# Toptachamann/Linear_Programming_Solver

Measured on AMD Instinct MI355X. Metric: simplex_pivots_per_sec, higher is better.
Workload: dtype f64

## Files before the change

### include/lpx.h

```cpp
#ifndef LPX_H
#define LPX_H

#include <stddef.h>
#include <stdint.h>

#ifdef __cplusplus
extern "C" {
#endif

#define LPX_ABI_VERSION 5

typedef enum lpx_status {
  LPX_OPTIMAL = 0,
  LPX_UNBOUNDED = 1,
  LPX_INFEASIBLE = 2,
  LPX_AUX_UNBOUNDED = 3,
  LPX_NO_DEGENERATE_PIVOT = 4,
  LPX_BAD_ARGUMENT = 5,
  LPX_RESTORE_INDEX_FAULT = 6,
  LPX_DEVICE_ERROR = 7,
  LPX_DIVIDE_BY_ZERO = 8,
  LPX_PIVOT_LIMIT = 9
} lpx_status;

// ... 31 lines not shown
  LPX_OPT_CHAIN_FENCES = 6,
  LPX_OPT_SWEEP_ROWS = 7,
  LPX_OPT_NT = 8,
  LPX_OPT_BATCH = 9,
  LPX_OPT_CHAIN_TRACE = 10,
  LPX_OPT_UPDATE_U = 11,
  LPX_OPT_UPDATE_ROWS = 12,
  LPX_OPT_A2_OFFSET = 13,
  LPX_OPT_SWEEP_FORM = 14,
  LPX_OPT_MULTI_ONEHOP = 15,
  LPX_OPT_SWEEP_CUS = 16,
  LPX_OPT_CHAIN_CUS = 17,
  LPX_OPT_FUSED = 18,
  LPX_OPT_CHAIN_FORM = 19,
  LPX_OPT_FIXUP_SIDE = 20,
  LPX_OPT_COUNT = 21
} lpx_option;
int lpx_state_set_option(lpx_state* s, int32_t key, int64_t value);
int lpx_state_get_option(const lpx_state* s, int32_t key, int64_t* value);

typedef struct lpx_state_info {
  int32_t block;
  int32_t chain_wgs;
  int32_t chain_wgs_requested;
  int32_t chain_resident_max;
  int32_t chain_blocks_per_cu;
  int32_t chain_stream_masked;
  int32_t chain_xcd_mask;
  int32_t sweep_xcd_mask;
  int32_t overlapped;
  int32_t nontemporal;
  int32_t sweep_rows;
  int32_t sweep_kernel;
  int32_t multi_onehop;
  int32_t sweep_clock_mhz;
  int32_t sweep_cus;
  int32_t arith_fused;
} lpx_state_info;
int lpx_state_get_info(lpx_state* s, lpx_state_info* out);
const char* lpx_sweep_kernel_name(int32_t code);
int lpx_state_read_chain_trace(lpx_state* s, int64_t* ticks, int32_t cap, int32_t* ndecisions);
int lpx_state_read_chain_trace_fine(lpx_state* s, int64_t* ticks, int32_t cap, int32_t* ndecisions, int32_t* stamps);

int lpx_state_set_block(lpx_state* s, int32_t pivots_per_sweep);
int lpx_state_get_block(const lpx_state* s);

int lpx_simplex_loop(lpx_state* s, int64_t max_pivots, int64_t* pivots_done, int32_t* status,
                     int32_t* track_slot);

int lpx_state_read(lpx_state* s, double* A, int64_t lda, double* b, double* c, double* v,
                   int32_t* perm);
int lpx_state_dims(const lpx_state* s, int32_t* m_local, int32_t* n, int32_t* row0, int32_t* m_global);
// ... 137 lines not shown
```

### linear_programming_solver_amd/_lib.py

```python
import ctypes as C
import os

_HERE = os.path.dirname(os.path.abspath(__file__))
LIB_PATH = os.environ.get("LPX_LIB_PATH") or os.path.join(_HERE, "liblpx.so")

OPTIMAL, UNBOUNDED, INFEASIBLE, AUX_UNBOUNDED, NO_DEGENERATE_PIVOT, BAD_ARGUMENT, RESTORE_INDEX_FAULT, \
    DEVICE_ERROR, DIVIDE_BY_ZERO, PIVOT_LIMIT = range(10)
CAND_HEADER = 8
BATCH_LDS_BYTES = 163840
ROUTES = ("cold", "primal", "dual")
PRICING = {"reference": 0, "first-positive": 0, "dantzig": 1, 0: 0, 1: 1}

OPTIONS = {"block": 0, "chain": 1, "overlap": 2, "overlap_serial": 3, "overlap_mask": 4, "chain_wgs": 5,
           "chain_fences": 6, "sweep_rows": 7, "nt": 8, "batch": 9, "chain_trace": 10, "update_u": 11,
           "update_rows": 12, "a2_offset": 13, "sweep_form": 14, "multi_onehop": 15, "sweep_cus": 16, "chain_cus": 17,
           "fused": 18, "chain_form": 19, "fixup_side": 20}

DEFAULT_FUSED = None


def set_default_arithmetic(mode):
    global DEFAULT_FUSED
    if mode not in ("auto", "plain", "fused"):
        raise ValueError('arithmetic mode is "auto", "plain" or "fused"')
    prev = "auto" if DEFAULT_FUSED is None else "fused" if DEFAULT_FUSED else "plain"
    DEFAULT_FUSED = None if mode == "auto" else mode == "fused"
    return prev


dp = C.POINTER(C.c_double)
ip = C.POINTER(C.c_int32)
# ... 8 lines not shown
        ("objective_rounded", C.c_double),
        ("objective_text", C.c_char * 64),
        ("pivots_phase1", C.c_int64),
        ("pivots_phase2", C.c_int64),
        ("x0_slot", C.c_int32),
        ("reserved", C.c_int32),
        ("seconds_total", C.c_double),
        ("seconds_pivots", C.c_double),
    ]


class StateInfo(C.Structure):
    _fields_ = [(k, C.c_int32) for k in (
        "block", "chain_wgs", "chain_wgs_requested", "chain_resident_max", "chain_blocks_per_cu",
        "chain_stream_masked", "chain_xcd_mask", "sweep_xcd_mask", "overlapped", "nontemporal", "sweep_rows",
        "sweep_kernel", "multi_onehop", "sweep_clock_mhz", "sweep_cus", "arith_fused")]


class SolveOptions(C.Structure):
    _fields_ = [
        ("device", C.c_int32),
        ("has_variable_names", C.c_int32),
        ("max_pivots", C.c_int64),
        ("restore_order", ip),
        ("perm_out", ip),
        ("x_out", dp),
        ("keep_state", C.POINTER(C.c_void_p)),
        ("pricing", C.c_int32),
        ("restore_order_len", C.c_int32),
        ("fused", C.c_int32),
        ("reserved", C.c_int32),
# ... 129 lines not shown
```

### linear_programming_solver_amd/csrc/lpx_decisions.inc

```
constexpr int kMaxBlock = 32;

__global__ __launch_bounds__(256) void k_peek_multi(const double* __restrict__ A, int64_t ld,
                                                    const double* __restrict__ b, int m_local, int row0,
                                                    const double* __restrict__ prow_ring,
                                                    const double* __restrict__ col_ring, int64_t mp,
                                                    const LpxCtl* __restrict__ ring, int np,
                                                    double* __restrict__ col_out, double* __restrict__ col0_out,
                                                    RatioRow* __restrict__ partial,
                                                    const LpxCtl* __restrict__ ctl) {
  __shared__ RatioRow sh[4];
  __shared__ double sh_pe[kMaxBlock], sh_p[kMaxBlock], sh_bl[kMaxBlock];
  __shared__ int sh_e[kMaxBlock], sh_l[kMaxBlock];
  if (ctl->status != kRunning) return;
  const int en = ctl->e_next;
  if (en < 0) return;
  if ((int)threadIdx.x < np) {
    const LpxCtl& q = ring[threadIdx.x];
    sh_e[threadIdx.x] = q.e_cur;
    sh_l[threadIdx.x] = q.l - row0;
    sh_p[threadIdx.x] = q.p;
    sh_bl[threadIdx.x] = q.bl;
    sh_pe[threadIdx.x] = prow_ring[(int64_t)threadIdx.x * ld + en];
  }
  __syncthreads();
// ... 214 lines not shown
  int dantzig, fences;
  LpxCtl* host_snap;
  long long* dbg;
  unsigned* census;
  int shard_row0;
  int m_global;
  int n_dev, dev;
  int mail_slot0;
  MgMail* mail_peer[kMaxDevices];
  double* prow_peer[kMaxDevices];
  unsigned long long* arrive_peer[kMaxDevices];
  int onehop;
  double* candrow_peer[kMaxDevices];
  unsigned long long* arrive2_peer[kMaxDevices];
  unsigned spin_max;
  int diag;
};

template <int KB>
__device__ __forceinline__ int chain_restart(const unsigned long long* sh_mask) {
  if constexpr (KB > 32) {
    const unsigned long long hi = sh_mask[1], lo = sh_mask[0];
    return hi ? 127 - __clzll((long long)hi) : (lo ? 63 - __clzll((long long)lo) : -1);
  } else {
    const unsigned long long lo = sh_mask[0];
    return lo ? 63 - __clzll((long long)lo) : -1;
  }
}

template <bool MG, int KB>
// ... 606 lines not shown
  for (int k = 1; k < NW; ++k) {
    const MinRec o = sh[slot][k];
    if (o.ratio < r.ratio || (o.ratio == r.ratio && o.row < r.row)) r = o;
  }
  a = r.a;
  b = r.b;
  return RatioRow{r.ratio, r.row, 0};
}

constexpr int kChain2Threads = 256;
#ifdef LPX_CHAIN2_OWN_WT
#define LPX_OWN_STORE(p_, x_) st_agent((p_), (x_))
#else
#define LPX_OWN_STORE(p_, x_) (*(p_) = (x_))
#endif
template <int KB, int NT, bool MG>
__device__ __forceinline__ void block_chain2_body(const ChainArgs& P) {
  static_assert(KB == 32 || KB == 64 || KB == 128, "ring half of 32, 64 or 128 slots");
  static_assert(NT % 64 == 0 && NT >= 256 && NT >= 2 * KB + (KB == 128 ? 0 : 64), "lanes for the pending pivots and the loader lane");
  static_assert(KB <= 64 || !MG, "the shards decide at most kShardBlockMax pivots per block");
  constexpr int NC = 2 * KB / 8;
  constexpr int NH = (2 * KB + 63) / 64;
  constexpr int kWin = 8;
  __shared__ RatioRow sh_rr[NT / 64];
  __shared__ MinRec sh_rec[2][NT / 64];
  __shared__ unsigned sh_part[kChainMaxWgs * 8], sh_hand[8];
  __shared__ __attribute__((aligned(16))) double sh_pe[2 * KB], sh_cs[2 * KB], sh_dv[2 * KB], sh_p[2 * KB], sh_bl[2 * KB];
  __shared__ __attribute__((aligned(16))) int sh_e[2 * KB], sh_l[2 * KB];
  __shared__ int sh_fail;
#ifdef LPX_CHAIN2_FINE
#define LPX_C2_STAMP(k) if (P.dbg && lead) P.dbg[s * 16 + (k)] = wall_clock64();
#define LPX_C2_STRIDE 16
#else
#define LPX_C2_STAMP(k)
#define LPX_C2_STRIDE 8
#endif
  const int row0 = MG ? P.shard_row0 : 0;
  const double* __restrict__ A = P.A;
  const double* __restrict__ b = P.b;
  const int64_t ld = P.ld, mp = P.mp;
  const int n = P.n, m = P.m, nb = P.nb, n_old = P.n_old;
  LpxCtl* const ctl = P.ctl;
#ifdef LPX_CHAIN2_ONE_XCD
  if (blockIdx.x & 7u) return;
  const unsigned bid = blockIdx.x >> 3;
  const int G = gridDim.x >> 3;
#else
  const unsigned bid = blockIdx.x;
  const int G = gridDim.x;
#endif
  const int T = G * NT, tid = threadIdx.x, gid = bid * NT + tid;
  const bool lead = gid == 0;
  const bool book = bid == (unsigned)(G - 1) && tid == 0;
  if (tid == 0) {
    sh_fail = 0;
    if (P.census) P.census[bid] = xcc_id() + 1u;
  }
#ifdef LPX_CHAIN2_LAUNCH_STAMPS
  long long* const lst = P.dbg ? P.dbg + 8 * kBlockMax + 8 * ((P.hand_base / (unsigned)kBlockMax) & 1u) : nullptr;
  if (lst && lead) { lst[0] = wall_clock64(); lst[3] = P.hand_base / (unsigned)kBlockMax; }
#endif
  if (lead) st_agent(reinterpret_cast<int32_t*>(P.bar_next), 0);
  int e = ctl->e_next;
  if (ctl->status != kRunning || e < 0 || nb < 1) {
    if (book && nb >= 1) P.up[0].do_update = 0;
    if (book) chain_publish(ctl, P.host_snap);
    return;
  }
  if (tid < 2 * KB) {
    sh_pe[tid] = 0.0; sh_cs[tid] = 0.0; sh_dv[tid] = 0.0; sh_p[tid] = 1.0; sh_bl[tid] = 0.0;
    sh_e[tid] = -1; sh_l[tid] = -1;
  }
  lds_barrier();
  if (tid < n_old) {
    const LpxCtl& q = P.up_o[tid];
    sh_e[tid] = q.e_cur; sh_l[tid] = q.l; sh_p[tid] = q.p; sh_bl[tid] = q.bl;
  }
  int64_t pivots = ctl->pivots;
  const int64_t max_pivots = ctl->max_pivots;
  double v = ctl->v;
  int track = ctl->track, parity = ctl->parity;
  unsigned target = 0;
// ... 151 lines not shown
      if constexpr (NC > 2 * kWin) {
        if (L_a > 2 * kWin) {
          load_window_a(i, 2 * kWin);
          ladder_a(2 * kWin);
        }
        if (L_a > 3 * kWin) {
          load_window_a(i, 3 * kWin);
          ladder_a(3 * kWin);
        }
      }
      if (Lo_a >= L_a) a_mid = a;
      P.col0[(int64_t)s * mp + i] = a_mid;
      LPX_C2_STAMP(9)
      st_agent(&P.col[(int64_t)s * mp + i], a);
      LPX_OWN_STORE(&P.own_col[(int64_t)s * mp + i], a);
      if (i == gid) { a_first = a; b_first = bi; }
      const double rt = ratio_of(a, bi);
      if (rt < best.ratio) {
        best = RatioRow{rt, ig, 0};
        best_a = a;
        best_b = bi;
      }
      i += T;
      __builtin_amdgcn_sched_barrier(0);
      if (i < m) load_row(i);
    }
    LPX_C2_STAMP(10)
    const double pc = from32(sh_hand[1], sh_hand[2]);
    const unsigned xtag = P.hand_base + (unsigned)s;
    {
// ... 11 lines not shown
      }
      for (int idx = tid; idx < G * 8; idx += NT) {
        if ((idx & 7) == 7) continue;
        unsigned long long g;
        unsigned spins = 0;
        while ((unsigned)((g = __hip_atomic_load(&gran[idx], __ATOMIC_RELAXED, __HIP_MEMORY_SCOPE_AGENT)) >> 32) != xtag) {
          LPX_BARRIER_SLEEP;
          if (++spins > P.spin_max) { sh_fail = 1; break; }
        }
        sh_part[idx] = (unsigned)g;
      }
      if (P.fences & 2) __builtin_amdgcn_fence(__ATOMIC_ACQUIRE, "agent");
      lds_barrier();
      if (sh_fail) {
        if (book) { ctl->status = 7 ; ctl->reserved = sh_fail + 1000 * s; chain_publish(ctl, P.host_snap); }
        return;
      }
    }
    if (P.dbg && lead) P.dbg[s * LPX_C2_STRIDE + 3] = wall_clock64();

    RatioRow mine = rr_none();
    double mine_a = 0.0, mine_b = 0.0;
    for (int t = tid & 63; t < G; t += 64) {
      const unsigned* q = &sh_part[t * 8];
      const RatioRow o{from32(q[0], q[1]), (int)q[6], 0};
      if (o.ratio < mine.ratio || (o.ratio == mine.ratio && o.row < mine.row)) {
        mine = o;
        mine_a = from32(q[2], q[3]);
        mine_b = from32(q[4], q[5]);
      }
    }
// ... 40 lines not shown
      w = rr_wave_min_all(theirs);
      win_p = 0.0; win_b = 0.0;
      if (w.row != INT_MAX) {
        const int wl = __ffsll((long long)__ballot(theirs.row == w.row)) - 1;
        win_p = lane_f64(theirs_a, wl);
        win_b = lane_f64(theirs_b, wl);
      }
      lds_barrier();
      if (sh_fail) { if (book) { ctl->status = 7; ctl->reserved = sh_fail + 1000 * s; chain_publish(ctl, P.host_snap); } return; }
    }
    if (w.row == INT_MAX || !(w.ratio < kInf)) {
      if (book) {
        ctl->status = 1; ctl->do_update = 0; ctl->l = -1; ctl->ratio = w.ratio; P.up[s].do_update = 0;
        chain_publish(ctl, P.host_snap);
      }
      return;
    }
    if (max_pivots >= 0 && pivots >= max_pivots) {
      if (book) {
        ctl->status = 9 ; ctl->do_update = 0; P.up[s].do_update = 0;
        chain_publish(ctl, P.host_snap);
      }
      return;
    }
    LPX_C2_STAMP(12)
    const int l = w.row;
    const double p = win_p, raw_b = win_b;
    if (p == 0.0) {
      if (book) { ctl->status = 8; ctl->do_update = 0; P.up[s].do_update = 0; chain_publish(ctl, P.host_snap); }
      return;
    }
    int rb;
    {
      unsigned long long hit[NH];
#pragma unroll
      for (int h = 0; h < NH; ++h) hit[h] = __ballot(sh_l[h * 64 + (tid & 63)] == l);
      rb = top_bit_of(hit);
    }
    const bool owner = !MG || (l >= row0 && l < row0 + m);
    const int ll = l - row0;
    const int fo_b = rb < 0 ? 0 : (rb < KB ? rb + 1 : n_old);
    const int fn_b = rb >= KB ? rb - KB + 1 : 0;
    const int co0_b = fo_b >> 3, co1_b = fo_b < n_old ? (n_old + 7) >> 3 : co0_b;
    const int cn0_b = fn_b >> 3, cn1_b = fn_b < s ? (s + 7) >> 3 : cn0_b;
    const int Lo_b = owner ? co1_b - co0_b : 0, L_b = owner ? Lo_b + (cn1_b - cn0_b) : 0;
// ... 208 lines not shown
    int e_next = -2;
    have_rec = false;
    if (window) {
      if (tid < 5) {
        unsigned long long rec = 0;
        unsigned spins = 0;
        for (;;) {
          rec = __hip_atomic_load(&hand[tid], __ATOMIC_RELAXED, __HIP_MEMORY_SCOPE_AGENT);
          if ((unsigned)(rec >> 32) == xtag) break;
          LPX_BARRIER_SLEEP;
          if (++spins > P.spin_max) { sh_fail = 4; break; }
        }
        sh_hand[tid] = (unsigned)rec;
      }
      lds_barrier();
      if (sh_fail) { if (book) { ctl->status = 7; ctl->reserved = sh_fail + 1000 * s; chain_publish(ctl, P.host_snap); } return; }
      e_next = (int)sh_hand[0] - 2;
      have_rec = e_next >= 0;
    }
    if (e_next < 0) {
      const RatioRow w2 = rr_block_min2(cand, sh_rr);
      if (tid == 0) {
        st_agent(&P.partB[bid].ratio, w2.ratio);
        st_agent(&P.partB[bid].row, w2.row);
      }
      target += (unsigned)G;
      if (!grid_barrier(P.bar, target, &sh_fail, P.fences, P.spin_max)) {
        if (book) { ctl->status = 7; chain_publish(ctl, P.host_snap); }
        return;
      }
      RatioRow m2 = rr_none();
      if (tid < G) { m2.ratio = ld_agent(&P.partB[tid].ratio); m2.row = ld_agent(&P.partB[tid].row); }
      const RatioRow w3 = rr_block_min2(m2, sh_rr);
      e_next = (w3.row == INT_MAX) ? -1 : w3.row;
    }
    if (P.dbg && lead) P.dbg[s * LPX_C2_STRIDE + 7] = wall_clock64();
    pivots += 1;
    parity ^= 1;
    if (book) {
      ctl->v = v; ctl->p = p; ctl->bl = bl; ctl->pc = pc; ctl->ratio = w.ratio;
      ctl->e_cur = e; ctl->l = l; ctl->e_next = e_next; ctl->parity = parity; ctl->pivots = pivots;
      ctl->track = track; ctl->do_update = 1;
      if (e_next < 0) {
        ctl->status = 0 ;
        if (s + 1 < nb) P.up[s + 1].do_update = 0;
      }
    }
    if (e_next < 0 || s + 1 == nb) {
      if (book) chain_publish(ctl, P.host_snap);
      return;
    }
    e = e_next;
    lds_barrier();
  }
}
template <int KB, int NT, bool MG>
__global__ __launch_bounds__(NT) void k_block_chain2_t(const ChainArgs P) {
  static_assert(KB == 32 || KB == 64, "ring half of 32 or 64 slots");
  block_chain2_body<KB, NT, MG>(P);
}
template <int NT>
__global__ __launch_bounds__(NT) void k_block_decide128(const ChainArgs P) {
  block_chain2_body<128, NT, false>(P);
}
#undef LPX_C2_STAMP
#undef LPX_C2_STRIDE
#undef LPX_CHAIN_STEP_A
#undef LPX_CHAIN_STEP_B
#undef LPX_CHAIN_CHUNK_A
#undef LPX_CHAIN_CHUNK_B
#undef LPX_CHAIN_LIVE
```

### linear_programming_solver_amd/csrc/lpx_engine.cpp

```cpp
#include <hip/hip_runtime.h>

#include <algorithm>
#include <chrono>
#include <cmath>
#include <cstdio>
#include <cstdlib>
#include <cstring>
#include <string>
#include <vector>

#include "../../include/lpx.h"
#include "lpx_kernels.h"
#include "lpx_internal.h"

using lpxk::Buffers;
using lpxk::Geometry;
using lpxk::LpxCtl;
using lpxk::RatioRow;

thread_local std::string g_last_error;

int fail(int status, const std::string& msg) {
  g_last_error = msg;
  return status;
// ... 35 lines not shown
    {"LPX_CHAIN_FENCES", 2, 0, 3},
    {"LPX_SWEEP_ROWS", 0, 0, 8192},
    {"LPX_NT", -1, -1, 1},
    {"LPX_BATCH", 0, 0, 4096},
    {"LPX_CHAIN_TRACE", 0, 0, 1},
    {"LPX_U", 1, 1, 4},
    {"LPX_ROWS_PER_TILE", 2, 2, 256},
    {"LPX_A2_OFFSET", 512, 0, 1 << 20},
    {"LPX_SWEEP_FORM", 0, 0, 4},
    {"LPX_MULTI_ONEHOP", 0, 0, 1},
    {"LPX_SWEEP_CUS", 0, 0, 256},
    {"LPX_CHAIN_CUS", 0, 0, 16},
    {"LPX_FUSED", 2, 0, 2},
    {"LPX_CHAIN_FORM", 1, 0, 1},
    {"LPX_FIXUP_SIDE", 4, 0, 4},
};

static const int64_t* env_defaults() {
  static int64_t d[LPX_OPT_COUNT];
  static const bool once = [] {
    for (int k = 0; k < LPX_OPT_COUNT; k++) {
      const OptionSpec& sp = kOptionSpec[k];
      int64_t v = sp.dflt;
      const char* e = getenv(sp.env);
      if (e && *e) v = std::max(sp.lo, std::min(sp.hi, (int64_t)atoll(e)));
      d[k] = v;
    }
    return true;
  }();
  (void)once;
// ... 573 lines not shown
lpxk::BlockRing ring_half(const lpx_state* s, int h) {
  lpxk::BlockRing R = s->R;
  const int64_t o = (int64_t)h * lpxk::kBlockMax;
  R.prow += o * s->B.ld;
  R.row0 += o * s->B.ld;
  R.col += o * R.mp;
  R.col0 += o * R.mp;
  if (R.fix_col) R.fix_col += o * R.mp;
  if (R.fix_row) R.fix_row += o * s->B.ld;
  if (R.col_packed) R.col_packed += (int64_t)h * (R.mp / 4 + 1) * (4 * lpxk::kColPackedRowBytes / sizeof(double));
  if (R.tickets) R.tickets += (int64_t)h * lpxk::sweep_ticket_slots(s->B.ld) * 32;
  R.up += o;
  return R;
}

#ifndef LPX_CHAIN_CUS_PER_XCD
#define LPX_CHAIN_CUS_PER_XCD 4
#endif
static int chain_cus_per_xcd(const lpx_state* s, int per_xcd) {
  int k = LPX_CHAIN_CUS_PER_XCD;
  const int64_t work = std::max<int64_t>(s->m, s->B.ld);
  const double bytes = 8.0 * (double)s->m * (double)s->B.ld;
  if (!s->multi_shard && work > 8192 && bytes <= 1.5 * 1073741824.0) k = 8;
  if (!s->multi_shard && work > 8192 && s->B.fused) k = 8;
  if (s->opt[LPX_OPT_CHAIN_CUS] > 0) k = std::max(4, (int)s->opt[LPX_OPT_CHAIN_CUS] / 4 * 4);
  return std::max(1, std::min(k, (per_xcd - 1) / 4 * 4));
}
int ensure_overlap_streams(lpx_state* s) {
  if (s->ov_chain) return 0;
  hipDeviceProp_t prop;
// ... 93 lines not shown
  double* Abuf[2] = {s->B.A, s->A2};
  double* bbuf[2] = {s->B.b, s->b2};
  int64_t decided = 0;
  int nb_prev = 0, nblk = 0;
  const bool serial = s->opt[LPX_OPT_OVERLAP_SERIAL] != 0;
  int fix_mode = serial ? 0 : (int)s->opt[LPX_OPT_FIXUP_SIDE];
  if (fix_mode == 4) fix_mode = 8.0 * (double)s->m * (double)s->B.ld >= 2.0 * 1073741824.0 ? 2 : 0;
  if (fix_mode > 0 && ensure_fix_side(s, fix_mode) != 0) {
    (void)hipGetLastError();
    fix_mode = 0;
  }
  auto issue_block = [&](int k) -> int {
    const int nb = block_len(K, max_pivots, decided);
    if (nb <= 0) return 1;
    const int h = k & 1;
    Buffers Brd = s->B;
    if (serial) {
      if (k >= 1) HIP_TRY(hipStreamWaitEvent(s->ov_chain, s->ev_ov_sweep[h ^ 1], 0));
      Brd.A = Abuf[h];
      Brd.b = bbuf[h];
      s->info.chain_wgs = lpxk::launch_block_chain(Brd, s->R, s->n, s->m, nb, h, h ^ 1, 0, 1, s->chain_seq++, s->pricing == 1,
                                                   chain_wgs, fences, trace, d_snap + h, s->ov_chain, nullptr, s->ev_ov_chain[h]);
    } else {
      if (k >= 2) HIP_TRY(hipStreamWaitEvent(s->ov_chain, s->ev_ov_sweep[h], 0));
      Brd.A = Abuf[k == 0 ? 0 : (k - 1) & 1];
      Brd.b = bbuf[k == 0 ? 0 : (k - 1) & 1];
      s->info.chain_wgs = lpxk::launch_block_chain(Brd, s->R, s->n, s->m, nb, h, h ^ 1, k > 0 ? nb_prev : 0, k == 0,
                                                   s->chain_seq++, s->pricing == 1, chain_wgs, fences, trace, d_snap + h,
                                                   s->ov_chain, nullptr, s->ev_ov_chain[h]);
    }
    s->chain_nb_last = nb;
    if (max_pivots >= 0 && decided == max_pivots) {
      decided += nb;
      return 0;
    }
    HIP_TRY(hipStreamWaitEvent(s->ov_sweep, s->ev_ov_chain[h], 0));
    Buffers Bdst = s->B;
    Bdst.A = Abuf[h ^ 1];
    Bdst.b = bbuf[h ^ 1];
    const lpxk::FixSide side{fix_mode > 0 ? s->ov_fix[fix_mode] : nullptr, s->ev_ov_chain[h], s->ev_ov_fix[h], s->ev_ov_pack[h]};
    if (int rc = launch_sweep_profiled(s, nb, s->ov_sweep, Bdst, ring_half(s, h), Abuf[h], bbuf[h], fix_mode > 0 ? &side : nullptr,
                                       s->ev_ov_sweep[h])) return rc;
    decided += nb;
    nb_prev = nb;
    nblk = k + 1;
    return 0;
  };
  int rc = issue_block(0);
  if (rc == 1) rc = 0;
  for (int k = 1; rc == 0; k++) {
    const int r = issue_block(k);
    if (r != 0 && r != 1) { rc = r; break; }
    hipError_t e = hipEventSynchronize(s->ev_ov_chain[(k - 1) & 1]);
    if (e != hipSuccess) { rc = fail(LPX_DEVICE_ERROR, hipGetErrorString(e)); break; }
    if (h2[(k - 1) & 1].status != lpxk::kRunning || r == 1) break;
  }
  (void)hipEventRecord(s->ev_ov_join[1], s->ov_chain);
// ... 27 lines not shown
  int64_t decided = 0;
  const bool fused = s->opt[LPX_OPT_CHAIN] != 0 && s->row0 == 0 && s->m == s->m_global;
  const int64_t work = std::max<int64_t>(s->m, s->B.ld);
  const int auto_wgs = (int)std::min<int64_t>(64, std::max<int64_t>(1, (work + 255) / 256));
  const int chain_wgs = fused ? clamp_chain_wgs(s, s->opt[LPX_OPT_CHAIN_WGS] > 0 ? (int)s->opt[LPX_OPT_CHAIN_WGS] : auto_wgs,
                                                device_cus(s))
                              : 0;
  const int fences = (int)s->opt[LPX_OPT_CHAIN_FENCES];
  const bool trace = s->opt[LPX_OPT_CHAIN_TRACE] != 0;
  s->info.chain_stream_masked = 0;
  s->info.overlapped = 0;
  LpxCtl* d_snap = nullptr;
  if (fused) HIP_TRY(hipHostGetDevicePointer((void**)&d_snap, s->h_snap, 0));
  auto issue_block = [&](int slot) -> int {
    const int nb = block_len(K, max_pivots, decided);
    if (fused && nb > 0) {
      s->info.chain_wgs = lpxk::launch_block_chain(s->B, s->R, s->n, s->m, nb, 0, 0, 0, 1, s->chain_seq++, s->pricing == 1,
                                                   chain_wgs, fences, trace, d_snap + slot, s->stream);
      s->chain_nb_last = nb;
    } else {
      for (int k = 0; k < nb; k++) {
        lpxk::launch_block_peek(s->B, s->R, s->n, s->m, s->row0, k, s->d_cand, s->stream);
        lpxk::launch_block_decide(s->B, s->R, s->n, s->m_global, s->d_cand, 1, k, s->stream);
        if (s->pricing == 1) lpxk::launch_entering_dantzig(s->B, s->n, false, s->stream);
      }
    }
    const bool probe_only = max_pivots >= 0 && decided == max_pivots;
    decided += nb;
    if (nb > 0 && !probe_only) {
      if (int rc = launch_sweep_profiled(s, nb)) return rc;
    }
    if (!fused)
      HIP_TRY(hipMemcpyAsync(&h2[slot], s->B.ctl, sizeof(LpxCtl), hipMemcpyDeviceToHost, s->stream));
    HIP_TRY(hipEventRecord(evs[slot], s->stream));
    return 0;
  };
  int rc = issue_block(0);
  int cur = 0;
  while (rc == 0) {
    rc = issue_block(cur ^ 1);
    if (rc) break;
    hipError_t e = hipEventSynchronize(evs[cur]);
    if (e != hipSuccess) { rc = fail(LPX_DEVICE_ERROR, hipGetErrorString(e)); break; }
    if (h2[cur].status != lpxk::kRunning) break;
    cur ^= 1;
// ... 76 lines not shown
    HIP_TRY(hipStreamSynchronize(s->stream));
    std::vector<unsigned> h(lpxk::kChainMaxWgs + 2);
    HIP_TRY(hipMemcpy(h.data(), s->R.census, h.size() * sizeof(unsigned), hipMemcpyDeviceToHost));
    for (int w = 0; w < s->info.chain_wgs && w < (int)lpxk::kChainMaxWgs; w++)
      if (h[w]) s->info.chain_xcd_mask |= 1 << ((h[w] - 1) & 15);
    s->info.sweep_xcd_mask = (int32_t)h[lpxk::kChainMaxWgs];
  }
  s->info.sweep_clock_mhz = 0;
  if (s->R.clk) {
    long long c32[32] = {};
    HIP_TRY(hipStreamSynchronize(s->stream));
    HIP_TRY(hipMemcpy(c32, s->R.clk, sizeof c32, hipMemcpyDeviceToHost));
    std::vector<double> mhz;
    for (int x = 0; x < 8; x++) {
      const long long* c4 = c32 + 4 * x;
      if (c4[3] > c4[1] && c4[2] > c4[0] && c4[3] - c4[1] > 1000) {
        const double f = 100.0 * (double)(c4[2] - c4[0]) / (double)(c4[3] - c4[1]);
        if (f > 300.0 && f < 3500.0) mhz.push_back(f);
      }
    }
    if (!mhz.empty()) {
      std::sort(mhz.begin(), mhz.end());
      s->info.sweep_clock_mhz = (int32_t)(mhz[mhz.size() / 2] + 0.5);
    }
  }
  *out = s->info;
  return 0;
}

extern "C" const char* lpx_sweep_kernel_name(int32_t code) { return lpxk::sweep_kernel_name(code); }

// ... 358 lines not shown
```

### linear_programming_solver_amd/csrc/lpx_kernels.h

```cpp
#pragma once
#include <hip/hip_runtime.h>
#include <stdint.h>

namespace lpxk {

constexpr int kRunning = -1;
constexpr double kEps = 1e-9;
constexpr double kInf = 1e50;

struct RatioRow {
  double ratio;
  int32_t row;
  int32_t pad;
};

struct LpxCtl {
  double v;
  double p;
  double bl;
  double pc;
  double ratio;
  int32_t e_next;
  int32_t e_cur;
  int32_t l;
// ... 46 lines not shown
  unsigned* chain_bar;
  double* chain_own_col;
  double* chain_own_prow;
  double* chain_own_dvc;
  double* chain_own_b;
  int32_t* chain_own_rs;
  long long* chain_dbg;
  unsigned* census;
  double* fix_col;
  double* fix_row;
  double* col_packed;
  unsigned* tickets;
  unsigned* sweep_fail;
  long long* clk;
  const double* zeros;
  void* mg_mail;
  unsigned long long* mg_arrive;
  double* mg_candrow;
  unsigned long long* mg_arrive2;
};
struct MgPeers {
  int n_dev, dev;
  int row0, m_global;
  int mail_slot0;
  void* mail[kMaxDevices];
  double* prow[kMaxDevices];
  unsigned long long* arrive[kMaxDevices];
  int onehop;
  double* candrow[kMaxDevices];
  unsigned long long* arrive2[kMaxDevices];
  unsigned spin_max;
};
enum SweepKernel { kSweepNone = 0, kSweepTiles = 1, kSweepMulti = 2, kSweepSteady = 3, kSweepPipe64 = 4, kSweepDma = 5, kSweepPull = 6, kSweepPull64 = 7, kSweepOne64 = 8, kSweepMfma64 = 9, kSweepMfma642 = 10, kSweepMfma128 = 11 };
struct FixSide { hipStream_t stream; hipEvent_t ready, done, packed; };
constexpr int kColPackedRowBytes = 1024;
constexpr int kSweep128Ranges = 3;
struct RestoreEntry { int32_t is_basic; int32_t index; double k; };

constexpr int kBatchLdsMax = 163840;
constexpr int kBatchScratchBytes = 512;
struct BatchLayout {
  int64_t ld, b, c, v, perm, image, col;
  int64_t lds_bytes;
};
__host__ __device__ inline BatchLayout batch_layout(int64_t m, int64_t n) {
  BatchLayout L;
  L.ld = n | 1;
  L.b = m * L.ld;
  L.c = L.b + m;
  L.v = L.c + n;
  L.perm = (L.v + 2) & ~(int64_t)1;
// ... 114 lines not shown
```

### linear_programming_solver_amd/csrc/lpx_kernels.hip

```cpp
#include "lpx_kernels.h"

#include <hip/hip_ext.h>

#include <atomic>

#include <limits.h>
#include <stdint.h>
#include <stdlib.h>

#include <algorithm>
#include <type_traits>

#ifndef LPX_FUSED
#define LPX_FUSED 0
#endif

namespace lpxk {
#if LPX_FUSED
namespace fused {
#else
namespace plain {
#endif

typedef double d2 __attribute__((ext_vector_type(2)));
// ... 812 lines not shown
  const int64_t ho = half * K, oo = old_half * K;
  P.prow = R.prow + ho * B.ld; P.col = R.col + ho * R.mp; P.col0 = R.col0 + ho * R.mp; P.row0 = R.row0 + ho * B.ld;
  P.own_col = R.chain_own_col + ho * R.mp; P.own_prow = R.chain_own_prow + ho * B.ld;
  P.own_dvc = R.chain_own_dvc + ho * R.mp; P.up = R.up + ho;
  P.prow_o = R.prow + oo * B.ld; P.col_o = R.col + oo * R.mp;
  P.own_col_o = R.chain_own_col + oo * R.mp; P.own_prow_o = R.chain_own_prow + oo * B.ld;
  P.own_dvc_o = R.chain_own_dvc + oo * R.mp; P.up_o = R.up + oo;
  P.n_old = n_old; P.own_b = R.chain_own_b; P.b_from_tableau = b_from_tableau; P.nb = nb;
  P.own_rs_a = R.chain_own_rs; P.own_rs_b = R.chain_own_rs + R.mp;
  P.partA = reinterpret_cast<ChainPart*>(R.chain_part_a); P.partB = reinterpret_cast<RatioRow*>(R.chain_part_b);
  P.bar = R.chain_bar + 32 * (seq & 1); P.bar_next = R.chain_bar + 32 * ((seq + 1) & 1);
  P.hand = reinterpret_cast<unsigned long long*>(R.chain_bar + 64);
  P.hand_base = (unsigned)(seq + 1) * (unsigned)kBlockMax;
  P.dantzig = dantzig; P.fences = fences; P.host_snap = host_snap; P.dbg = trace ? R.chain_dbg : nullptr;
  P.spin_max = (mg && mg->spin_max) ? mg->spin_max : (1u << 22);
#ifdef LPX_DIAG_BUILD
  static const int chain_diag = getenv("LPX_CHAIN_DIAG") ? atoi(getenv("LPX_CHAIN_DIAG")) : 0;
  P.diag = chain_diag;
#endif
  P.census = R.census;
  if (mg) {
    P.shard_row0 = mg->row0; P.m_global = mg->m_global; P.n_dev = mg->n_dev; P.dev = mg->dev;
    P.mail_slot0 = mg->mail_slot0;
    P.onehop = mg->onehop;
    for (int d = 0; d < mg->n_dev && d < kMaxDevices; ++d) {
      P.mail_peer[d] = reinterpret_cast<MgMail*>(mg->mail[d]);
      P.prow_peer[d] = mg->prow[d] + ho * B.ld;
      P.arrive_peer[d] = mg->arrive[d];
      P.candrow_peer[d] = mg->candrow[d];
      P.arrive2_peer[d] = mg->arrive2[d];
// ... 85 lines not shown
#undef LPX_PRE_ONE64
#if LPX_FUSED
    hipLaunchKernelGGL(k_pack_multipliers_mfma, dim3(1), dim3(256), 0, s, R.col, R.mp, R.up, 0, 0, R.col_packed, R.tickets, 0, (long long*)nullptr, 0);
#ifdef LPX_WITH_VARIANTS
#define LPX_PRE_MFMA64(NT_, OOP_) \
    hipLaunchKernelGGL((k_sweep64_mfma<NT_, OOP_>), dim3(1), dim3(256), 0, s, A, A, ld, 0, R.prow, R.up, 0, 1, R.col_packed, R.tickets);
    LPX_EACH_NT_OOP(LPX_PRE_MFMA64)
#undef LPX_PRE_MFMA64
#endif
#define LPX_PRE_MFMA642(NT_, OOP_) \
    hipLaunchKernelGGL((k_sweep64_mfma2<NT_, OOP_>), dim3(1), dim3(256), 0, s, A, A, ld, 0, R.prow, R.up, 0, 1, R.col_packed, R.tickets, 33, (long long*)nullptr);
    LPX_EACH_NT_OOP(LPX_PRE_MFMA642)
#undef LPX_PRE_MFMA642
    hipLaunchKernelGGL(k_pack_multipliers_mfma128, dim3(1), dim3(256), 0, s, R.col, R.mp, R.up, 0, 0, R.col_packed, R.tickets, 0, (long long*)nullptr);
#define LPX_PRE_MFMA128(NT_, OOP_) \
    hipLaunchKernelGGL((k_sweep128_mfma<NT_, OOP_>), dim3(1), dim3(256), 0, s, A, A, ld, 0, R.prow, R.up, 0, 0, R.col_packed, R.tickets, 1);
    LPX_EACH_NT_OOP(LPX_PRE_MFMA128)
#undef LPX_PRE_MFMA128
#endif
  }
#undef LPX_PRE_PULL
#undef LPX_PRE_DMA
#undef LPX_PRE_PIPE
#undef LPX_PRE_STEADY
#undef LPX_PRE_MULTI
#undef LPX_PRE_T32
#undef LPX_PRE_T16
#undef LPX_PRE_T8
#undef LPX_PRE_T4
#undef LPX_PRE_T2
#undef LPX_PRE_TILES
// ... 135 lines not shown
  if (A_src) { if (nt) LPX_LAUNCH_MFMA64(true, true); else LPX_LAUNCH_MFMA64(false, true); }
  else { if (nt) LPX_LAUNCH_MFMA64(true, false); else LPX_LAUNCH_MFMA64(false, false); }
#undef LPX_LAUNCH_MFMA64
#else
  (void)G;
#endif
}
#endif

#if LPX_FUSED
static void launch_sweep128_mfma(const Buffers& B, const BlockRing& R, int m_local, int kmax, bool nt, const double* A_src,
                                 hipStream_t s, int cus, const FixSide* side, hipEvent_t t0, hipEvent_t t1) {
  const int nsub = (int)(B.ld / 64);
  const int ntiles = m_local / 16;
  const int nranges = std::max(1, std::min(kSweep128Ranges, ntiles));
  LPX_LAUNCH_STOP(k_pack_multipliers_mfma128, dim3(ntiles), dim3(256), pack_stream(side, s), pack_stop(side), R.col, R.mp, R.up, kmax,
                  ntiles, R.col_packed, R.tickets, 1 + nsub * nranges, R.clk);
  pack_done(side, s);
  const dim3 grid(std::max(1, std::min(2 * cus, nsub * nranges))), block(256);
#define LPX_LAUNCH_MFMA128(NT_, OOP_)                                                                                    \
  LPX_LAUNCH_TIMED((k_sweep128_mfma<NT_, OOP_>), grid, block, s, t0, t1, B.A, A_src, B.ld, m_local, R.prow, R.up, kmax, nsub, \
                   R.col_packed, R.tickets, nranges)
  if (A_src) { if (nt) LPX_LAUNCH_MFMA128(true, true); else LPX_LAUNCH_MFMA128(false, true); }
  else { if (nt) LPX_LAUNCH_MFMA128(true, false); else LPX_LAUNCH_MFMA128(false, false); }
#undef LPX_LAUNCH_MFMA128
}
#endif

static int choose_sweep_rows(int m_local, int64_t ld, int K, int cus) {
  const int64_t nstrips = (ld + 511) / 512;
  const int64_t slots = std::max(1, 2 * cus);
  const int prologue_rows = std::max(8, (K * 3) / 2);
  int best_rows = kSweepChunk;
  int64_t best_cost = INT64_MAX;
  const int max_rows = (int)std::min<int64_t>(4096, (((int64_t)1 << 32) - 1) / (ld * 8) / kSweepChunk * kSweepChunk);
  for (int rows = kSweepChunk; rows <= std::max(kSweepChunk, max_rows); rows += kSweepChunk) {
    const int64_t groups = (m_local + rows - 1) / rows;
// ... 52 lines not shown
  else side = nullptr;
  if (K <= 16) {
    bracket();
    int rows_per_tile = rows_per_wg <= 0 ? 16 : rows_per_wg;
    rows_per_tile = std::max(8, std::min(rows_per_tile, kSweepMaxRows)) & ~7;
    while (rows_per_tile > 8 && (int64_t)rows_per_tile * B.ld * 8 >= (int64_t)1 << 32) rows_per_tile -= 8;
    if (K <= 2) launch_sweep_tiles<2>(B, R, m_local, K, rows_per_tile, nt, A_src, s);
    else if (K <= 4) launch_sweep_tiles<4>(B, R, m_local, K, rows_per_tile, nt, A_src, s);
    else if (K <= 8) launch_sweep_tiles<8>(B, R, m_local, K, rows_per_tile, nt, A_src, s);
    else launch_sweep_tiles<16>(B, R, m_local, K, rows_per_tile, nt, A_src, s);
    rows_per_wg = rows_per_tile;
    used = kSweepTiles;
  } else if (K > 64) {
    bool mfma128 = false;
#if LPX_FUSED
    mfma128 = form != 3 && m_local % 16 == 0 && m_local >= 16 && B.ld % 512 == 0 && 16 * B.ld * 8 + 1024 < ((int64_t)1 << 32) &&
              R.tickets && R.col_packed;
#endif
    if (mfma128) {
#if LPX_FUSED
      timed_own = before_sweep && after_sweep;
      if (!timed_own) bracket();
      launch_sweep128_mfma(B, R, m_local, K, nt, A_src, s, cus, side, timed_own ? before_sweep : nullptr, timed_own ? after_sweep : nullptr);
#endif
      rows_per_wg = 16;
      used = kSweepMfma128;
    } else {
      bracket();
      int rows = choose_sweep_rows(m_local, B.ld, 32, cus);
      while (rows > kSweepChunk && (int64_t)rows * B.ld * 8 >= (int64_t)1 << 32) rows -= kSweepChunk;
      for (int slot0 = 0; slot0 < K; slot0 += 32) launch_sweep_k<32>(B, R, m_local, K, rows, nt, slot0 == 0 ? A_src : nullptr, s, 0, slot0);
      rows_per_wg = rows;
// ... 160 lines not shown
```

### linear_programming_solver_amd/csrc/lpx_sweeps.inc

```
constexpr int kSweepMaxRows = 128;
#ifndef LPX_SWEEP_NBUF
#define LPX_SWEEP_NBUF 2
#endif

__device__ __forceinline__ int ring_count(const LpxCtl* __restrict__ ring, int kcap, int kmax, int* sh_np) {
  if (threadIdx.x < 64) {
    const int lane = threadIdx.x;
    const bool ok = lane < kcap && lane < kmax && ring[lane].do_update != 0;
    const unsigned long long mask = __ballot(ok);
    if (lane == 0) *sh_np = (~mask == 0ull) ? 64 : (__ffsll((long long)~mask) - 1);
  }
  __syncthreads();
  return *sh_np;
}
__device__ __forceinline__ int ring_count128(const LpxCtl* __restrict__ ring, int kmax, int* sh_np) {
  if (threadIdx.x < 64) {
    const int lane = threadIdx.x;
    const unsigned long long m0 = __ballot(lane < kmax && ring[lane].do_update != 0);
    const unsigned long long m1 = __ballot(lane + 64 < kmax && ring[lane + 64].do_update != 0);
    const int n0 = (~m0 == 0ull) ? 64 : (__ffsll((long long)~m0) - 1);
    const int n1 = (~m1 == 0ull) ? 64 : (__ffsll((long long)~m1) - 1);
    if (lane == 0) *sh_np = n0 < 64 ? n0 : 64 + n1;
  }
  __syncthreads();
// ... 912 lines not shown
  for (int q = 0; q < 8; ++q) {
    const int idx = q * 256 + threadIdx.x;
    const int g = idx >> 6, l = idx & 63, k = l >> 4, i = l & 15;
    const int s = 4 * g + k;
    const double c = s < np ? col_ring[(int64_t)s * mp + (int64_t)tile * 16 + i] : 0.0;
    colM[(int64_t)tile * 2048 + (g >> 1) * 128 + 2 * l + (g & 1)] = -c;
  }
}
#define LPX_MFMA_FENCE __builtin_amdgcn_sched_barrier(0)
template <bool NT, bool OOP>
__global__ __launch_bounds__(256, 2) void k_sweep128_mfma(double* A, const double* Asrc,
                                                          int64_t ld, int m_local,
                                                          const double* __restrict__ prow_ring,
                                                          const LpxCtl* __restrict__ ring, int kmax, int nsub,
                                                          const double* colM,
                                                          unsigned* tickets, int nranges) {
  constexpr int NG = 32, CT = 4;
  constexpr int kRsrcWord3 = 0x00020000;
  constexpr int kAuxNt = NT ? 2 : 0;
  __shared__ __attribute__((aligned(16))) double sh_b[NG * CT * 64];
  __shared__ int sh_np, sh_chunk;
  const int np = ring_count128(ring, kmax, &sh_np);
  if (np < 1 && !OOP) return;
  const int lane = threadIdx.x & 63;
  const int wave = __builtin_amdgcn_readfirstlane((int)(threadIdx.x >> 6));
  const int rowblocks = m_local / 16;
  const int per_range = (rowblocks + nranges - 1) / nranges;
  const int nchunks = nsub * nranges;
  const int64_t row_bytes = ld * 8;
  const uint32_t rb32 = (uint32_t)row_bytes;
  const uint32_t off_c = (uint32_t)(lane >> 4) * rb32 + (uint32_t)(lane & 15) * 8u;
  const uint32_t off_a = (uint32_t)lane * 8u;
  int sub_loaded = -1;
  for (;;) {
    if (threadIdx.x == 0) sh_chunk = (int)atomicAdd(tickets, 1u);
    __syncthreads();
    const int chunk = __builtin_amdgcn_readfirstlane(sh_chunk);
    if (chunk >= nchunks) return;
    const int sub = chunk % nsub, range = chunk / nsub;
    const int rb0 = range * per_range;
    const int ntiles = min(rowblocks, rb0 + per_range) - rb0;
    if (sub != sub_loaded) {
      for (int q = wave; q < NG * CT; q += 4) {
        const int g = q / CT, ct = q % CT;
        const int s = 4 * g + (lane >> 4);
        sh_b[q * 64 + lane] = s < np ? prow_ring[(int64_t)s * ld + sub * 64 + ct * 16 + (lane & 15)] : 0.0;
      }
      sub_loaded = sub;
    }
    __syncthreads();
    if (ntiles > 0) {
      unsigned* const ctr = tickets + 32 * (1 + chunk);
      char* const dst_base = reinterpret_cast<char*>(A + sub * 64) + (int64_t)rb0 * 16 * row_bytes;
// ... 351 lines not shown
```

Baseline: 24470.

## Pack MFMA multipliers inside the decide chain kernel instead of a separate pack launch

When the fused chain form runs a 128-slot block on a single shard, the decide kernel now writes each negated pivot column directly into the packed MFMA column layout and resets the sweep tickets. On early exit it pads the unused slots with zeros. This lets the sweep skip the separate k_pack_multipliers_mfma128 launch and its stream/event handoff. In exchange, every column element costs an extra scattered store inside the latency-critical chain kernel. The change also moves clock sampling from the pack kernel into the sweep kernel and tightens a filter in the clock-rate estimate.

Result: no change. 24280 (-0.8%).

```diff
diff --git a/include/lpx.h b/include/lpx.h
--- a/include/lpx.h
+++ b/include/lpx.h
@@ -69,7 +69,8 @@
   LPX_OPT_FUSED = 18,
   LPX_OPT_CHAIN_FORM = 19,
   LPX_OPT_FIXUP_SIDE = 20,
-  LPX_OPT_COUNT = 21
+  LPX_OPT_PACK_IN_DECIDE = 21,
+  LPX_OPT_COUNT = 22
 } lpx_option;
 int lpx_state_set_option(lpx_state* s, int32_t key, int64_t value);
 int lpx_state_get_option(const lpx_state* s, int32_t key, int64_t* value);
@@ -91,6 +92,8 @@
   int32_t sweep_clock_mhz;
   int32_t sweep_cus;
   int32_t arith_fused;
+  int32_t pack_in_decide;
+  int32_t reserved;
 } lpx_state_info;
 int lpx_state_get_info(lpx_state* s, lpx_state_info* out);
 const char* lpx_sweep_kernel_name(int32_t code);
diff --git a/linear_programming_solver_amd/_lib.py b/linear_programming_solver_amd/_lib.py
--- a/linear_programming_solver_amd/_lib.py
+++ b/linear_programming_solver_amd/_lib.py
@@ -14,7 +14,7 @@
 OPTIONS = {"block": 0, "chain": 1, "overlap": 2, "overlap_serial": 3, "overlap_mask": 4, "chain_wgs": 5,
            "chain_fences": 6, "sweep_rows": 7, "nt": 8, "batch": 9, "chain_trace": 10, "update_u": 11,
            "update_rows": 12, "a2_offset": 13, "sweep_form": 14, "multi_onehop": 15, "sweep_cus": 16, "chain_cus": 17,
-           "fused": 18, "chain_form": 19, "fixup_side": 20}
+           "fused": 18, "chain_form": 19, "fixup_side": 20, "pack_in_decide": 21}
 
 DEFAULT_FUSED = None
 
@@ -53,7 +53,7 @@
     _fields_ = [(k, C.c_int32) for k in (
         "block", "chain_wgs", "chain_wgs_requested", "chain_resident_max", "chain_blocks_per_cu",
         "chain_stream_masked", "chain_xcd_mask", "sweep_xcd_mask", "overlapped", "nontemporal", "sweep_rows",
-        "sweep_kernel", "multi_onehop", "sweep_clock_mhz", "sweep_cus", "arith_fused")]
+        "sweep_kernel", "multi_onehop", "sweep_clock_mhz", "sweep_cus", "arith_fused", "pack_in_decide", "reserved")]
 
 
 class SolveOptions(C.Structure):
diff --git a/linear_programming_solver_amd/csrc/lpx_decisions.inc b/linear_programming_solver_amd/csrc/lpx_decisions.inc
--- a/linear_programming_solver_amd/csrc/lpx_decisions.inc
+++ b/linear_programming_solver_amd/csrc/lpx_decisions.inc
@@ -252,6 +252,9 @@
   double* candrow_peer[kMaxDevices];
   unsigned long long* arrive2_peer[kMaxDevices];
   unsigned spin_max;
+  double* colM;
+  unsigned* tickets;
+  int nctr;
   int diag;
 };
 
@@ -888,6 +891,14 @@
 #else
 #define LPX_OWN_STORE(p_, x_) (*(p_) = (x_))
 #endif
+__device__ __forceinline__ int64_t colm_index(int s, int i) {
+  return (int64_t)(i >> 4) * 2048 + (s >> 3) * 128 + 2 * ((s & 3) * 16 + (i & 15)) + ((s >> 2) & 1);
+}
+__device__ __forceinline__ void colm_pad(double* colM, int done, int gid, int T, int m) {
+  if (!colM || done >= 128) return;
+  for (int i = gid; i < m; i += T)
+    for (int u = done; u < 128; ++u) colM[colm_index(u, i)] = -0.0;
+}
 template <int KB, int NT, bool MG>
 __device__ __forceinline__ void block_chain2_body(const ChainArgs& P) {
   static_assert(KB == 32 || KB == 64 || KB == 128, "ring half of 32, 64 or 128 slots");
@@ -909,6 +920,7 @@
 #define LPX_C2_STAMP(k)
 #define LPX_C2_STRIDE 8
 #endif
+#define LPX_C2_LEAVE(done_) do { if constexpr (KB == 128) colm_pad(P.colM, (done_), gid, T, m); return; } while (0)
   const int row0 = MG ? P.shard_row0 : 0;
   const double* __restrict__ A = P.A;
   const double* __restrict__ b = P.b;
@@ -935,11 +947,15 @@
   if (lst && lead) { lst[0] = wall_clock64(); lst[3] = P.hand_base / (unsigned)kBlockMax; }
 #endif
   if (lead) st_agent(reinterpret_cast<int32_t*>(P.bar_next), 0);
+  if constexpr (KB == 128) {
+    if (P.colM && bid == 0)
+      for (int u = tid; u < P.nctr; u += NT) P.tickets[u * 32] = 0u;
+  }
   int e = ctl->e_next;
   if (ctl->status != kRunning || e < 0 || nb < 1) {
     if (book && nb >= 1) P.up[0].do_update = 0;
     if (book) chain_publish(ctl, P.host_snap);
-    return;
+    LPX_C2_LEAVE(0);
   }
   if (tid < 2 * KB) {
     sh_pe[tid] = 0.0; sh_cs[tid] = 0.0; sh_dv[tid] = 0.0; sh_p[tid] = 1.0; sh_bl[tid] = 0.0;
@@ -1121,6 +1137,9 @@
       LPX_C2_STAMP(9)
       st_agent(&P.col[(int64_t)s * mp + i], a);
       LPX_OWN_STORE(&P.own_col[(int64_t)s * mp + i], a);
+      if constexpr (KB == 128) {
+        if (P.colM) P.colM[colm_index(s, i)] = -a;
+      }
       if (i == gid) { a_first = a; b_first = bi; }
       const double rt = ratio_of(a, bi);
       if (rt < best.ratio) {
@@ -1162,7 +1181,7 @@
       lds_barrier();
       if (sh_fail) {
         if (book) { ctl->status = 7 ; ctl->reserved = sh_fail + 1000 * s; chain_publish(ctl, P.host_snap); }
-        return;
+        LPX_C2_LEAVE(s);
       }
     }
     if (P.dbg && lead) P.dbg[s * LPX_C2_STRIDE + 3] = wall_clock64();
@@ -1233,21 +1252,21 @@
         ctl->status = 1; ctl->do_update = 0; ctl->l = -1; ctl->ratio = w.ratio; P.up[s].do_update = 0;
         chain_publish(ctl, P.host_snap);
       }
-      return;
+      LPX_C2_LEAVE(s);
     }
     if (max_pivots >= 0 && pivots >= max_pivots) {
       if (book) {
         ctl->status = 9 ; ctl->do_update = 0; P.up[s].do_update = 0;
         chain_publish(ctl, P.host_snap);
       }
-      return;
+      LPX_C2_LEAVE(s);
     }
     LPX_C2_STAMP(12)
     const int l = w.row;
     const double p = win_p, raw_b = win_b;
     if (p == 0.0) {
       if (book) { ctl->status = 8; ctl->do_update = 0; P.up[s].do_update = 0; chain_publish(ctl, P.host_snap); }
-      return;
+      LPX_C2_LEAVE(s);
     }
     int rb;
     {
@@ -1486,7 +1505,7 @@
         sh_hand[tid] = (unsigned)rec;
       }
       lds_barrier();
-      if (sh_fail) { if (book) { ctl->status = 7; ctl->reserved = sh_fail + 1000 * s; chain_publish(ctl, P.host_snap); } return; }
+      if (sh_fail) { if (book) { ctl->status = 7; ctl->reserved = sh_fail + 1000 * s; chain_publish(ctl, P.host_snap); } LPX_C2_LEAVE(s + 1); }
       e_next = (int)sh_hand[0] - 2;
       have_rec = e_next >= 0;
     }
@@ -1499,7 +1518,7 @@
       target += (unsigned)G;
       if (!grid_barrier(P.bar, target, &sh_fail, P.fences, P.spin_max)) {
         if (book) { ctl->status = 7; chain_publish(ctl, P.host_snap); }
-        return;
+        LPX_C2_LEAVE(s + 1);
       }
       RatioRow m2 = rr_none();
       if (tid < G) { m2.ratio = ld_agent(&P.partB[tid].ratio); m2.row = ld_agent(&P.partB[tid].row); }
@@ -1520,7 +1539,7 @@
     }
     if (e_next < 0 || s + 1 == nb) {
       if (book) chain_publish(ctl, P.host_snap);
-      return;
+      LPX_C2_LEAVE(s + 1);
     }
     e = e_next;
     lds_barrier();
@@ -1535,6 +1554,7 @@
 __global__ __launch_bounds__(NT) void k_block_decide128(const ChainArgs P) {
   block_chain2_body<128, NT, false>(P);
 }
+#undef LPX_C2_LEAVE
 #undef LPX_C2_STAMP
 #undef LPX_C2_STRIDE
 #undef LPX_CHAIN_STEP_A
diff --git a/linear_programming_solver_amd/csrc/lpx_engine.cpp b/linear_programming_solver_amd/csrc/lpx_engine.cpp
--- a/linear_programming_solver_amd/csrc/lpx_engine.cpp
+++ b/linear_programming_solver_amd/csrc/lpx_engine.cpp
@@ -73,6 +73,7 @@
     {"LPX_FUSED", 2, 0, 2},
     {"LPX_CHAIN_FORM", 1, 0, 1},
     {"LPX_FIXUP_SIDE", 4, 0, 4},
+    {"LPX_PACK_IN_DECIDE", 1, 0, 1},
 };
 
 static const int64_t* env_defaults() {
@@ -676,6 +677,13 @@
   return R;
 }
 
+static int set_pack_in_decide(lpx_state* s, int nb) {
+  const bool on = s->opt[LPX_OPT_PACK_IN_DECIDE] != 0 && s->B.chain_form == 1 && s->row0 == 0 && s->m == s->m_global &&
+                  lpxk::sweep128_whole(s->B.fused != 0, s->B.ld, s->R, s->m, nb, (int)s->opt[LPX_OPT_SWEEP_FORM]);
+  s->R.pack_in_decide = on ? 1 : 0;
+  return s->R.pack_in_decide;
+}
+
 #ifndef LPX_CHAIN_CUS_PER_XCD
 #define LPX_CHAIN_CUS_PER_XCD 4
 #endif
@@ -799,6 +807,7 @@
     const int nb = block_len(K, max_pivots, decided);
     if (nb <= 0) return 1;
     const int h = k & 1;
+    const int packed = set_pack_in_decide(s, nb);
     Buffers Brd = s->B;
     if (serial) {
       if (k >= 1) HIP_TRY(hipStreamWaitEvent(s->ov_chain, s->ev_ov_sweep[h ^ 1], 0));
@@ -826,6 +835,7 @@
     const lpxk::FixSide side{fix_mode > 0 ? s->ov_fix[fix_mode] : nullptr, s->ev_ov_chain[h], s->ev_ov_fix[h], s->ev_ov_pack[h]};
     if (int rc = launch_sweep_profiled(s, nb, s->ov_sweep, Bdst, ring_half(s, h), Abuf[h], bbuf[h], fix_mode > 0 ? &side : nullptr,
                                        s->ev_ov_sweep[h])) return rc;
+    s->info.pack_in_decide = packed;
     decided += nb;
     nb_prev = nb;
     nblk = k + 1;
@@ -883,7 +893,9 @@
   if (fused) HIP_TRY(hipHostGetDevicePointer((void**)&d_snap, s->h_snap, 0));
   auto issue_block = [&](int slot) -> int {
     const int nb = block_len(K, max_pivots, decided);
+    s->R.pack_in_decide = 0;
     if (fused && nb > 0) {
+      set_pack_in_decide(s, nb);
       s->info.chain_wgs = lpxk::launch_block_chain(s->B, s->R, s->n, s->m, nb, 0, 0, 0, 1, s->chain_seq++, s->pricing == 1,
                                                    chain_wgs, fences, trace, d_snap + slot, s->stream);
       s->chain_nb_last = nb;
@@ -898,6 +910,7 @@
     decided += nb;
     if (nb > 0 && !probe_only) {
       if (int rc = launch_sweep_profiled(s, nb)) return rc;
+      s->info.pack_in_decide = s->R.pack_in_decide;
     }
     if (!fused)
       HIP_TRY(hipMemcpyAsync(&h2[slot], s->B.ctl, sizeof(LpxCtl), hipMemcpyDeviceToHost, s->stream));
@@ -1004,7 +1017,7 @@
     std::vector<double> mhz;
     for (int x = 0; x < 8; x++) {
       const long long* c4 = c32 + 4 * x;
-      if (c4[3] > c4[1] && c4[2] > c4[0] && c4[3] - c4[1] > 1000) {
+      if (c4[0] > 0 && c4[1] > 0 && c4[3] > c4[1] && c4[2] > c4[0] && c4[3] - c4[1] > 1000) {
         const double f = 100.0 * (double)(c4[2] - c4[0]) / (double)(c4[3] - c4[1]);
         if (f > 300.0 && f < 3500.0) mhz.push_back(f);
       }
diff --git a/linear_programming_solver_amd/csrc/lpx_kernels.h b/linear_programming_solver_amd/csrc/lpx_kernels.h
--- a/linear_programming_solver_amd/csrc/lpx_kernels.h
+++ b/linear_programming_solver_amd/csrc/lpx_kernels.h
@@ -84,6 +84,7 @@
   unsigned* sweep_fail;
   long long* clk;
   const double* zeros;
+  int pack_in_decide;
   void* mg_mail;
   unsigned long long* mg_arrive;
   double* mg_candrow;
@@ -105,6 +106,10 @@
 struct FixSide { hipStream_t stream; hipEvent_t ready, done, packed; };
 constexpr int kColPackedRowBytes = 1024;
 constexpr int kSweep128Ranges = 3;
+inline bool sweep128_whole(bool fused, int64_t ld, const BlockRing& R, int m_local, int K, int form) {
+  return fused && K > 64 && K <= kBlockMax && form != 3 && m_local % 16 == 0 && m_local >= 16 && ld % 512 == 0 &&
+         16 * ld * 8 + 1024 < ((int64_t)1 << 32) && R.tickets && R.col_packed;
+}
 struct RestoreEntry { int32_t is_basic; int32_t index; double k; };
 
 constexpr int kBatchLdsMax = 163840;
diff --git a/linear_programming_solver_amd/csrc/lpx_kernels.hip b/linear_programming_solver_amd/csrc/lpx_kernels.hip
--- a/linear_programming_solver_amd/csrc/lpx_kernels.hip
+++ b/linear_programming_solver_amd/csrc/lpx_kernels.hip
@@ -850,6 +850,11 @@
   P.hand_base = (unsigned)(seq + 1) * (unsigned)kBlockMax;
   P.dantzig = dantzig; P.fences = fences; P.host_snap = host_snap; P.dbg = trace ? R.chain_dbg : nullptr;
   P.spin_max = (mg && mg->spin_max) ? mg->spin_max : (1u << 22);
+  if (R.pack_in_decide && form2 && mg == nullptr && nb > 64 && m % 16 == 0 && R.col_packed && R.tickets) {
+    P.colM = R.col_packed + (int64_t)half * (R.mp / 4 + 1) * (4 * kColPackedRowBytes / sizeof(double));
+    P.tickets = R.tickets + (int64_t)half * sweep_ticket_slots(B.ld) * 32;
+    P.nctr = 1 + (int)(B.ld / 64) * std::max(1, std::min(kSweep128Ranges, m / 16));
+  }
 #ifdef LPX_DIAG_BUILD
   static const int chain_diag = getenv("LPX_CHAIN_DIAG") ? atoi(getenv("LPX_CHAIN_DIAG")) : 0;
   P.diag = chain_diag;
@@ -965,7 +970,7 @@
 #undef LPX_PRE_MFMA642
     hipLaunchKernelGGL(k_pack_multipliers_mfma128, dim3(1), dim3(256), 0, s, R.col, R.mp, R.up, 0, 0, R.col_packed, R.tickets, 0, (long long*)nullptr);
 #define LPX_PRE_MFMA128(NT_, OOP_) \
-    hipLaunchKernelGGL((k_sweep128_mfma<NT_, OOP_>), dim3(1), dim3(256), 0, s, A, A, ld, 0, R.prow, R.up, 0, 0, R.col_packed, R.tickets, 1);
+    hipLaunchKernelGGL((k_sweep128_mfma<NT_, OOP_>), dim3(1), dim3(256), 0, s, A, A, ld, 0, R.prow, R.up, 0, 0, R.col_packed, R.tickets, 1, (long long*)nullptr);
     LPX_EACH_NT_OOP(LPX_PRE_MFMA128)
 #undef LPX_PRE_MFMA128
 #endif
@@ -1131,13 +1136,15 @@
   const int nsub = (int)(B.ld / 64);
   const int ntiles = m_local / 16;
   const int nranges = std::max(1, std::min(kSweep128Ranges, ntiles));
-  LPX_LAUNCH_STOP(k_pack_multipliers_mfma128, dim3(ntiles), dim3(256), pack_stream(side, s), pack_stop(side), R.col, R.mp, R.up, kmax,
-                  ntiles, R.col_packed, R.tickets, 1 + nsub * nranges, R.clk);
-  pack_done(side, s);
+  if (!R.pack_in_decide) {
+    LPX_LAUNCH_STOP(k_pack_multipliers_mfma128, dim3(ntiles), dim3(256), pack_stream(side, s), pack_stop(side), R.col, R.mp, R.up, kmax,
+                    ntiles, R.col_packed, R.tickets, 1 + nsub * nranges, (long long*)nullptr);
+    pack_done(side, s);
+  }
   const dim3 grid(std::max(1, std::min(2 * cus, nsub * nranges))), block(256);
 #define LPX_LAUNCH_MFMA128(NT_, OOP_)                                                                                    \
   LPX_LAUNCH_TIMED((k_sweep128_mfma<NT_, OOP_>), grid, block, s, t0, t1, B.A, A_src, B.ld, m_local, R.prow, R.up, kmax, nsub, \
-                   R.col_packed, R.tickets, nranges)
+                   R.col_packed, R.tickets, nranges, R.clk)
   if (A_src) { if (nt) LPX_LAUNCH_MFMA128(true, true); else LPX_LAUNCH_MFMA128(false, true); }
   else { if (nt) LPX_LAUNCH_MFMA128(true, false); else LPX_LAUNCH_MFMA128(false, false); }
 #undef LPX_LAUNCH_MFMA128
@@ -1220,8 +1227,7 @@
   } else if (K > 64) {
     bool mfma128 = false;
 #if LPX_FUSED
-    mfma128 = form != 3 && m_local % 16 == 0 && m_local >= 16 && B.ld % 512 == 0 && 16 * B.ld * 8 + 1024 < ((int64_t)1 << 32) &&
-              R.tickets && R.col_packed;
+    mfma128 = sweep128_whole(true, B.ld, R, m_local, K, form);
 #endif
     if (mfma128) {
 #if LPX_FUSED
diff --git a/linear_programming_solver_amd/csrc/lpx_sweeps.inc b/linear_programming_solver_amd/csrc/lpx_sweeps.inc
--- a/linear_programming_solver_amd/csrc/lpx_sweeps.inc
+++ b/linear_programming_solver_amd/csrc/lpx_sweeps.inc
@@ -950,12 +950,15 @@
                                                           const double* __restrict__ prow_ring,
                                                           const LpxCtl* __restrict__ ring, int kmax, int nsub,
                                                           const double* colM,
-                                                          unsigned* tickets, int nranges) {
+                                                          unsigned* tickets, int nranges,
+                                                          long long* __restrict__ clk = nullptr) {
   constexpr int NG = 32, CT = 4;
   constexpr int kRsrcWord3 = 0x00020000;
   constexpr int kAuxNt = NT ? 2 : 0;
   __shared__ __attribute__((aligned(16))) double sh_b[NG * CT * 64];
   __shared__ int sh_np, sh_chunk;
+  __shared__ long long sh_front[2];
+  if (clk && blockIdx.x < 16 && threadIdx.x == 0) { sh_front[0] = __builtin_amdgcn_s_memtime(); sh_front[1] = wall_clock64(); }
   const int np = ring_count128(ring, kmax, &sh_np);
   if (np < 1 && !OOP) return;
   const int lane = threadIdx.x & 63;
@@ -972,7 +975,14 @@
     if (threadIdx.x == 0) sh_chunk = (int)atomicAdd(tickets, 1u);
     __syncthreads();
     const int chunk = __builtin_amdgcn_readfirstlane(sh_chunk);
-    if (chunk >= nchunks) return;
+    if (chunk >= nchunks) {
+      if (clk && blockIdx.x < 16 && threadIdx.x == 0) {
+        const unsigned x = xcc_id() & 7u;
+        clk[x * 4 + 0] = sh_front[0]; clk[x * 4 + 1] = sh_front[1];
+        clk[x * 4 + 2] = __builtin_amdgcn_s_memtime(); clk[x * 4 + 3] = wall_clock64();
+      }
+      return;
+    }
     const int sub = chunk % nsub, range = chunk / nsub;
     const int rb0 = range * per_range;
     const int ntiles = min(rowblocks, rb0 + per_range) - rb0;
```
